# sara-nl/saraGAN

Measured on AMD Instinct MI355X. Metric: 3D volumes/sec/node (G+D step) at 128x128x32, higher is better.
Workload: dtype bf16

## Files before the change

### saragan_amd/csrc/common.h

```cpp
#pragma once
#include <hip/hip_runtime.h>
#include <stdint.h>
#include <mutex>
#include "../../include/saragan_hip.h"

typedef __bf16 bf16_t;
typedef float f32x4 __attribute__((ext_vector_type(4)));
typedef float f32x16 __attribute__((ext_vector_type(16)));
typedef __bf16 bf16x8 __attribute__((ext_vector_type(8)));
typedef __bf16 bf16x4 __attribute__((ext_vector_type(4)));
typedef short s16x4 __attribute__((ext_vector_type(4)));
typedef uint32_t u32x4 __attribute__((ext_vector_type(4)));

#define SG_STORE16_GUARD(v) asm volatile("s_nop 1" ::"v"(v))
typedef uint32_t u32x2 __attribute__((ext_vector_type(2)));

#define SG_LAUNCH_CHECK()                          \
  do {                                             \
    hipError_t e__ = hipGetLastError();            \
    if (e__ != hipSuccess) return (int)e__;        \
  } while (0)

static inline hipStream_t sg_st(sg_stream_t s) { return (hipStream_t)s; }

struct sg_config {
  int fwd_lds, fwd_tg;
  int fwd_v1, fwd_no_pw, fwd_no_dense;
  int fwd_no_v3, fwd_no_v3s, fwd_no_v4, fwd_no_v5, fwd_no_ksplit;
  int fwd3p_16;
  int fwd3s_16;
  int fwd_no_3p;
  int fwd3_gx, fwd3_no_lean;
  int fwd4_gx, fwd4_no_lean, fwd4_no_wres;
  int wgrad_v1, wgrad_no_v3, wgrad_no_lean;
  int wgrad_no_w16;
  int wgrad3l_min_cols;
  int wgrad3l_16;
  int wgrad_v1_blocks;
  int dbg_flags;
  int no_small;
  int deterministic;
  int gemm_ks_model;
  int gemm_k333_maxvox;
  int no_gemm;
};
const sg_config& sg_cfg();

bool sg_gemm_conv_eligible(const sg_conv_shape* s, sg_dtype dt);
size_t sg_gemm_conv_workspace(const sg_conv_shape* s, sg_dtype dt);
int sg_gemm_conv_fwd(const void* x, const void* wp, void* y, const sg_conv_shape* s, const float* bias, int act, float slope,
                     const uint32_t* mask_bits, float mask_slope, uint32_t* sign_out, void* workspace, size_t workspace_bytes,
                     hipStream_t st, bool* used);

bool sg_small_eligible(const sg_conv_shape* s);
bool sg_small_wgrad_eligible(const sg_conv_shape* s);
size_t sg_small_tail_bytes(const sg_conv_shape* s);
size_t sg_small_wgrad_workspace(const sg_conv_shape* s);
int sg_small_pack(const float* w, float coef, int flip, void* tail, const sg_conv_shape* s, sg_dtype dt, hipStream_t st);
int sg_small_fwd(const void* x, const void* tail, void* y, const sg_conv_shape* s, const float* bias, int act, float slope,
                 int pixel_norm, float eps, float* pn_scale, const uint32_t* mask_bits, float mask_slope, uint32_t* sign_out,
                 sg_dtype dt, hipStream_t st);
int sg_small_wgrad(const void* x, const void* dy, float* dw, float* dbias, float coef, void* workspace, size_t workspace_bytes,
                   const sg_conv_shape* s, sg_dtype dt, hipStream_t st);

#define SG_ALLOW_160K_LDS(kern)                                                                                  \
  do {                                                                                                           \
    static std::once_flag once__;                                                                                \
    static hipError_t err__ = hipSuccess;                                                                        \
    std::call_once(once__, [&] {                                                                                 \
      err__ = hipFuncSetAttribute((const void*)(kern), hipFuncAttributeMaxDynamicSharedMemorySize, 160 * 1024);  \
    });                                                                                                          \
    if (err__ != hipSuccess) return (int)err__;                                                                  \
  } while (0)
static inline size_t sg_esize(sg_dtype dt) { return dt == SG_BF16 ? 2 : 4; }
static inline bool sg_aligned16(const void* p) { return (((uintptr_t)p) & 15) == 0; }

__device__ __forceinline__ void philox4x32_10(uint32_t c0, uint32_t c1, uint32_t c2, uint32_t c3, uint32_t k0,
// ... 244 lines not shown
```

### saragan_amd/csrc/conv3d.hip

```cpp
#include "common.h"
#include "prof.h"
#include "conv_args.h"

struct PackArgs {
  const float* w;
  void* wp;
  float coef;
  int taps, kd, kh, kw, cin, cout, nchunk, ntile, flip;
};

template <typename T>
__global__ void pack_weights_kernel(PackArgs a) {
  constexpr int CH = sg_traits<T>::CH;
  constexpr int EPL = CH / 2;
  const int64_t total = (int64_t)a.nchunk * a.taps * a.ntile * 64 * EPL;
  T* out = reinterpret_cast<T*>(a.wp);
  for (int64_t i = (int64_t)blockIdx.x * blockDim.x + threadIdx.x; i < total; i += (int64_t)gridDim.x * blockDim.x) {
    int e = (int)(i % EPL);
    int64_t q = i / EPL;
    int lane = (int)(q % 64); q /= 64;
    int nt = (int)(q % a.ntile); q /= a.ntile;
    int tap = (int)(q % a.taps);
    int chunk = (int)(q / a.taps);
    int ci = chunk * CH + (lane >> 5) * EPL + e;
// ... 11 lines not shown
  }
}

constexpr int SG_PACK_BATCH = 56;
struct PackBatchArgs {
  PackArgs item[SG_PACK_BATCH];
};

template <typename T>
__global__ void pack_weights_batch_kernel(PackBatchArgs b) {
  const PackArgs& a = b.item[blockIdx.y];
  constexpr int CH = sg_traits<T>::CH;
  constexpr int EPL = CH / 2;
  const int64_t total = (int64_t)a.nchunk * a.taps * a.ntile * 64 * EPL;
  T* out = reinterpret_cast<T*>(a.wp);
  for (int64_t i = (int64_t)blockIdx.x * blockDim.x + threadIdx.x; i < total; i += (int64_t)gridDim.x * blockDim.x) {
    int e = (int)(i % EPL);
    int64_t q = i / EPL;
    int lane = (int)(q % 64); q /= 64;
    int nt = (int)(q % a.ntile); q /= a.ntile;
    int tap = (int)(q % a.taps);
    int chunk = (int)(q / a.taps);
    int ci = chunk * CH + (lane >> 5) * EPL + e;
    int co = nt * 32 + (lane & 31);
    float v = 0.f;
    if (ci < a.cin && co < a.cout) {
      v = a.flip ? a.w[((int64_t)(a.taps - 1 - tap) * a.cout + co) * a.cin + ci] : a.w[((int64_t)tap * a.cin + ci) * a.cout + co];
      v *= a.coef;
    }
    out[i] = sg_traits<T>::from_f(v);
  }
}

static inline int conv_nchunk(const sg_conv_shape* s, sg_dtype dt) {
  int ch = dt == SG_BF16 ? 16 : 8;
  return sg_cdiv(s->cin, ch);
}
static inline int conv_ntile(const sg_conv_shape* s) { return sg_cdiv(s->cout, 32); }

static int conv_shape_ok(const sg_conv_shape* s) {
  if (!s) return 0;
  if (s->n < 1 || s->d < 1 || s->h < 1 || s->w < 1 || s->cin < 1 || s->cout < 1) return 0;
  const bool sub = s->kd == 2 && s->kh == 2 && s->kw == 2 && !s->upsample_in;
  if (s->kd < 1 || s->kh < 1 || s->kw < 1 || (!sub && (!(s->kd & 1) || !(s->kh & 1) || !(s->kw & 1)))) return 0;
  if (s->kd > 7 || s->kh > 7 || s->kw > 7) return 0;
  if (s->upsample_in && ((s->d | s->h | s->w) & 1)) return 0;
  return 1;
}

extern "C" size_t sg_conv3d_packed_bytes(const sg_conv_shape* s, sg_dtype dt) {
  if (!conv_shape_ok(s)) return 0;
  return (size_t)conv_nchunk(s, dt) * (s->kd * s->kh * s->kw) * conv_ntile(s) * 1024 + sg_small_tail_bytes(s) + sg_pack16_bytes(s, dt);
}

extern "C" int sg_conv3d_pack_weights(const float* w, float coef, int transpose_flip, void* wp,
                                      const sg_conv_shape* s, sg_dtype dt, sg_stream_t st) {
  if (!conv_shape_ok(s) || !w || !wp) return SG_EINVAL;
  PackArgs a;
  a.w = w; a.wp = wp; a.coef = coef;
  a.kd = s->kd; a.kh = s->kh; a.kw = s->kw; a.taps = s->kd * s->kh * s->kw;
  a.cin = s->cin; a.cout = s->cout; a.nchunk = conv_nchunk(s, dt); a.ntile = conv_ntile(s);
  a.flip = transpose_flip ? 1 : 0;
  int64_t total = (int64_t)a.nchunk * a.taps * a.ntile * 64 * (dt == SG_BF16 ? 8 : 4);
  int blocks = (int)((total + 255) / 256);
  if (blocks > 4096) blocks = 4096;
  if (dt == SG_BF16)
    hipLaunchKernelGGL(pack_weights_kernel<bf16_t>, dim3(blocks), dim3(256), 0, sg_st(st), a);
  else
    hipLaunchKernelGGL(pack_weights_kernel<float>, dim3(blocks), dim3(256), 0, sg_st(st), a);
  SG_LAUNCH_CHECK();
  if (sg_pack16_bytes(s, dt)) {
    void* tail = reinterpret_cast<char*>(wp) + (size_t)a.nchunk * a.taps * a.ntile * 1024;
    return sg_pack16_batch(1, &w, &coef, &a.flip, &tail, s, sg_st(st));
  }
  if (sg_small_tail_bytes(s))
    return sg_small_pack(w, coef, a.flip, reinterpret_cast<char*>(wp) + (size_t)a.nchunk * a.taps * a.ntile * 1024, s, dt, sg_st(st));
  return SG_OK;
}

extern "C" int sg_conv3d_pack_weights_batch(int n, const float* const* w, const float* coef, const int* transpose_flip,
                                            void* const* wp, const sg_conv_shape* shapes, sg_dtype dt, sg_stream_t st) {
  if (n < 0 || (n > 0 && (!w || !coef || !transpose_flip || !wp || !shapes))) return SG_EINVAL;
  if (dt != SG_BF16 && dt != SG_F32) return SG_EINVAL;
  for (int i = 0; i < n; ++i)
    if (!conv_shape_ok(&shapes[i]) || !w[i] || !wp[i]) return SG_EINVAL;
  for (int i0 = 0; i0 < n; i0 += SG_PACK_BATCH) {
    const int m = n - i0 < SG_PACK_BATCH ? n - i0 : SG_PACK_BATCH;
    PackBatchArgs b;
    int64_t most = 0;
    for (int j = 0; j < SG_PACK_BATCH; ++j) {
      const int i = i0 + (j < m ? j : 0);
      const sg_conv_shape* s = &shapes[i];
      PackArgs& a = b.item[j];
      a.w = w[i]; a.wp = wp[i]; a.coef = coef[i];
      a.kd = s->kd; a.kh = s->kh; a.kw = s->kw; a.taps = s->kd * s->kh * s->kw;
      a.cin = s->cin; a.cout = s->cout; a.nchunk = conv_nchunk(s, dt); a.ntile = conv_ntile(s);
      a.flip = transpose_flip[i] ? 1 : 0;
      const int64_t total = (int64_t)a.nchunk * a.taps * a.ntile * 64 * (dt == SG_BF16 ? 8 : 4);
      if (j < m && total > most) most = total;
    }
    int blocks = (int)((most + 255) / 256);
    if (blocks > 256) blocks = 256;
    if (blocks < 1) blocks = 1;
    if (dt == SG_BF16)
      hipLaunchKernelGGL(pack_weights_batch_kernel<bf16_t>, dim3((unsigned)blocks, (unsigned)m), dim3(256), 0, sg_st(st), b);
    else
      hipLaunchKernelGGL(pack_weights_batch_kernel<float>, dim3((unsigned)blocks, (unsigned)m), dim3(256), 0, sg_st(st), b);
    SG_LAUNCH_CHECK();
  }
  constexpr int M16 = 64;
  const float* w16[M16]; float c16[M16]; int f16[M16]; void* d16[M16]; sg_conv_shape s16[M16];
  int n16 = 0;
  for (int i = 0; i < n; ++i) {
    const sg_conv_shape* s = &shapes[i];
    char* tail = reinterpret_cast<char*>(wp[i]) + (size_t)conv_nchunk(s, dt) * (s->kd * s->kh * s->kw) * conv_ntile(s) * 1024;
    int rc = SG_OK;
    if (sg_pack16_bytes(s, dt)) {
      w16[n16] = w[i]; c16[n16] = coef[i]; f16[n16] = transpose_flip[i] ? 1 : 0; d16[n16] = tail; s16[n16] = *s;
      if (++n16 == M16) {
        rc = sg_pack16_batch(n16, w16, c16, f16, d16, s16, sg_st(st));
        n16 = 0;
      }
    } else if (sg_small_tail_bytes(s)) rc = sg_small_pack(w[i], coef[i], transpose_flip[i] ? 1 : 0, tail, s, dt, sg_st(st));
    if (rc != SG_OK) return rc;
  }
  if (n16) return sg_pack16_batch(n16, w16, c16, f16, d16, s16, sg_st(st));
  return SG_OK;
}


template <typename T> struct sg_vec4 { typedef u32x4 type; };
template <> struct sg_vec4<bf16_t> { typedef u32x2 type; };

template <typename T, int MTW, int NTB>
__device__ __forceinline__ void conv_epilogue(f32x16 (&acc)[MTW][NTB], const int64_t (&ooff)[MTW],
                                              const ConvFwdArgs& a, int nt0, int hh) {
  T* y = reinterpret_cast<T*>(a.y);
// ... 2385 lines not shown
    for (int u = 0; u < U; ++u) acc = sg_mfma_chunk<T>(wf[u], xf[u], acc);
  }
#pragma unroll
  for (int i = 0; i < 16; ++i) red[wave][i][lane] = acc[i];
  __syncthreads();
  if (wave == 0) {
#pragma unroll
    for (int i = 0; i < 16; ++i) {
      float t = 0.f;
#pragma unroll
      for (int w = 0; w < 16; ++w) t += red[w][i][lane];
      const int co = nt0 * 32 + (i & 3) + 8 * (i >> 2) + 4 * hh;
      if (a.bias != nullptr && co < a.cout) t += a.bias[co];
      if (a.act) t = fmaxf(t, t * a.slope);
      acc[i] = t;
    }
    if (a.sign_out != nullptr) {
      const uint32_t sw = sg_sign_word(acc, hh);
      if (hh == 0 && vlive) a.sign_out[(int64_t)vrow * a.ntile + nt0] = sw;
    }
    if (a.mask_bits != nullptr && vlive) sg_apply_sign_word(acc, a.mask_bits[(int64_t)vrow * a.ntile + nt0], hh, a.mask_slope);
    if (vlive) {
      T* yrow = reinterpret_cast<T*>(a.y) + (int64_t)vrow * a.cout;
#pragma unroll
      for (int i = 0; i < 16; ++i) {
        const int co = nt0 * 32 + (i & 3) + 8 * (i >> 2) + 4 * hh;
        if (co < a.cout) yrow[co] = sg_traits<T>::from_f(acc[i]);
      }
    }
  }
}

template <typename T>
static int launch_pw_fwd(ConvFwdArgs& a, const sg_conv_shape* s, hipStream_t st, bool* used) {
  *used = false;
  constexpr int E = 16 / (int)sizeof(T);
  if (a.taps != 1 || s->upsample_in || a.pixel_norm) return SG_OK;
  const int64_t nvox = (int64_t)s->n * s->d * s->h * s->w;
  if (nvox <= 128 && s->cin % sg_traits<T>::CH == 0 && a.nchunk >= 64 && !sg_cfg().fwd_no_dense) {
    SG_KNAME("dense_small_m<%s>", sg_tname<T>());
    hipLaunchKernelGGL(dense_small_m_kernel<T>, dim3((unsigned)a.ntile, (unsigned)((nvox + 31) / 32)), dim3(1024), 0, st, a, (int)nvox);
    SG_LAUNCH_CHECK();
    *used = true;
    return SG_OK;
  }
  if (s->cin <= 4 && s->cout % E == 0 && 256 % (s->cout / E) == 0 && s->cout / E <= 256 &&
      ((s->cout / E) & (s->cout / E - 1)) == 0) {
    const int rows = 256 / (s->cout / E);
    const int64_t full = (nvox + rows - 1) / rows;
    int64_t nb = (full + 7) / 8;
    if (nb < 2048) nb = full < 2048 ? full : 2048;
    SG_KNAME("pw_fwd_small_cin<%s>", sg_tname<T>());
    switch (s->cin) {
      case 1: hipLaunchKernelGGL((pw_fwd_small_cin_kernel<T, 1>), dim3((unsigned)nb), dim3(256), 0, st, a, nvox); break;
      case 2: hipLaunchKernelGGL((pw_fwd_small_cin_kernel<T, 2>), dim3((unsigned)nb), dim3(256), 0, st, a, nvox); break;
      case 3: hipLaunchKernelGGL((pw_fwd_small_cin_kernel<T, 3>), dim3((unsigned)nb), dim3(256), 0, st, a, nvox); break;
      default: hipLaunchKernelGGL((pw_fwd_small_cin_kernel<T, 4>), dim3((unsigned)nb), dim3(256), 0, st, a, nvox); break;
    }
    SG_LAUNCH_CHECK();
    *used = true;
  } else if (s->cout <= 4 && s->cin % E == 0 && (s->cin / E) <= 64 && ((s->cin / E) & (s->cin / E - 1)) == 0) {
    const int rows = 256 / (s->cin / E);
    int64_t nb = (nvox + rows - 1) / rows;
    if (nb > 8192) nb = 8192;
    SG_KNAME("pw_fwd_small_cout<%s>", sg_tname<T>());
    hipLaunchKernelGGL(pw_fwd_small_cout_kernel<T>, dim3((unsigned)nb), dim3(256), 0, st, a, nvox);
    SG_LAUNCH_CHECK();
    *used = true;
  }
  return SG_OK;
}

unsigned long long* g_dbg_ts = nullptr;
extern "C" __attribute__((visibility("default"))) void sg_debug_set_ts_buffer(void* p) { g_dbg_ts = (unsigned long long*)p; }

extern "C" size_t sg_conv3d_pw_epilogue_workspace(void) { return (size_t)SG_PW_PART_ROWS * 64 * sizeof(float); }

extern "C" size_t sg_conv3d_fwd_workspace(const sg_conv_shape* s, sg_dtype dt) {
  if (!conv_shape_ok(s) || dt != SG_BF16) return 0;
  if (!sg_cfg().no_gemm && sg_gemm_conv_eligible(s, dt)) return sg_gemm_conv_workspace(s, dt);
  if (s->kd == 3 && s->kh == 3 && s->kw == 3 && s->cin == 64 && s->cout == 32 && s->w % 32 == 0 && s->d >= 4 &&
      (!s->upsample_in || ((s->d | s->h | s->w) & 1) == 0))
    return (size_t)s->n * s->d * s->h * s->w * (size_t)s->cout * 4;
  return 0;
}

extern "C" int sg_conv3d_fwd(const void* x, const void* wp, void* y, const sg_conv_shape* s,
                             const sg_conv_epilogue* ep, sg_dtype dt, sg_stream_t st) {
  if (!conv_shape_ok(s) || !x || !wp || (!y && !(ep && ep->pw_x))) return SG_EINVAL;
  if (ep && ep->struct_size != (uint32_t)sizeof(sg_conv_epilogue)) return SG_EINVAL;
  if (!sg_aligned16(x) || !sg_aligned16(wp) || !sg_aligned16(y)) return SG_EALIGN;
  ConvFwdArgs a;
  a.x = x; a.wp = wp; a.y = y;
  a.bias = ep ? ep->bias : nullptr;
  a.pn_scale = ep ? ep->pn_scale : nullptr;
  a.mask_bits = ep ? reinterpret_cast<const uint32_t*>(ep->mask_bits) : nullptr;
  a.sign_out = ep ? reinterpret_cast<uint32_t*>(ep->sign_out) : nullptr;
  a.mask_slope = ep ? ep->mask_slope : 0.f;
  a.act = ep ? ep->act : 0;
  a.slope = ep ? ep->slope : 0.f;
  a.pixel_norm = ep ? ep->pixel_norm : 0;
  a.eps = ep ? ep->eps : 0.f;
  a.tap_d = ep ? ep->tap_off[0] : 0; a.tap_h = ep ? ep->tap_off[1] : 0; a.tap_w = ep ? ep->tap_off[2] : 0;
  a.pool = ep ? ep->pool : 0;
  if (a.pool < 0 || a.pool > 3) return SG_EINVAL;
  a.pnb_y = ep ? ep->pn_bwd_y : nullptr;
  a.pnb_scale = ep ? ep->pn_bwd_scale : nullptr;
  if ((a.pnb_y != nullptr) != (a.pnb_scale != nullptr) || (a.pnb_y && !sg_aligned16(a.pnb_y))) return SG_EINVAL;
  a.xcs = s->cin; a.xco = 0; a.addend = nullptr;
  a.in_mask = ep ? reinterpret_cast<const uint32_t*>(ep->in_mask_bits) : nullptr;
  a.in_mask_slope = ep ? ep->in_mask_slope : 0.f;
  a.in_gain = ep ? ep->in_gain : 1.f;
// ... 39 lines not shown
    return rc;
  }
  if (a.pool && (subpixel || dt != SG_BF16 || sg_cfg().fwd_v1 || (s->cin * 2) % 16 != 0 || a.pixel_norm ||
                 (a.pool == 1 && (sg_cfg().fwd_no_v3 || sg_cfg().fwd_no_v3s)) || (a.pool == 2 && sg_cfg().fwd_no_v5) ||
                 (a.pool == 3 && (s->cin != 32 || s->kd != 3 || s->kh != 3 || s->kw != 3 || s->upsample_in || !sg_cfg().fwd3s_16 ||
                                  sg_cfg().fwd_no_v3 || sg_cfg().fwd_no_v3s || (ep && ep->x_plane_channels)))))
    return SG_EUNSUPPORTED;
  if (a.pnb_y && (subpixel || dt != SG_BF16 || sg_cfg().fwd_v1 || sg_cfg().fwd_no_v3 || sg_cfg().fwd_no_v3s || a.pool ||
                  a.pixel_norm || (s->cin * 2) % 16 != 0 || s->kd != 3 || s->kh != 3 || s->kw != 3 || s->upsample_in ||
                  (ep && ep->x_plane_channels)))
    return SG_EUNSUPPORTED;
  if (sg_small_eligible(s) && !sg_cfg().no_small && !a.pool && !a.pnb_y && !(ep && ep->x_plane_channels)) {
    rc = sg_small_fwd(x, reinterpret_cast<const char*>(wp) + (size_t)a.nchunk * a.taps * a.ntile * 1024, y, s, a.bias, a.act, a.slope,
                      a.pixel_norm, a.eps, a.pn_scale, a.mask_bits, a.mask_slope, a.sign_out, dt, hs);
    prof.done(rc);
    return rc;
  }
  if (dt == SG_BF16 && !sg_cfg().no_gemm && !a.pool && !a.pnb_y && !a.pixel_norm && !(ep && ep->x_plane_channels) &&
      sg_gemm_conv_eligible(s, dt)) {
    bool used = false;
    rc = sg_gemm_conv_fwd(x, wp, y, s, a.bias, a.act, a.slope, a.mask_bits, a.mask_slope, a.sign_out, ep ? ep->workspace : nullptr,
                          ep ? ep->workspace_bytes : 0, hs, &used);
    if (rc != SG_OK || used) { prof.done(rc); return rc; }
  }
  if (a.pool == 2) {
    bool used = false;
    rc = launch_fwd5(a, s, hs, &used);
    if (rc == SG_OK && !used) rc = SG_EUNSUPPORTED;
    prof.done(rc);
    return rc;
  }
  if (!sg_cfg().fwd_no_pw && !a.pool && !a.pnb_y) {
    bool used = false;
    rc = dt == SG_BF16 ? launch_pw_fwd<bf16_t>(a, s, hs, &used) : launch_pw_fwd<float>(a, s, hs, &used);
    if (rc != SG_OK || used) { prof.done(rc); return rc; }
  }
  const bool v2 = ((s->cin * es) % 16 == 0) && !sg_cfg().fwd_v1;
  const int xpl = ep ? ep->x_plane_channels : 0;
  if (xpl != 0 && (xpl != 32 || s->upsample_in || a.pool || !(v2 && !sg_cfg().fwd_no_v3 && (!a.pixel_norm || a.ntile == 1)))) {
    prof.done(xpl != 32 ? SG_EINVAL : SG_EUNSUPPORTED);
    return xpl != 32 ? SG_EINVAL : SG_EUNSUPPORTED;
  }
  if (v2 && !sg_cfg().fwd_no_v3 && (!a.pixel_norm || a.ntile == 1)) {
    bool used = false;
    rc = SG_OK;
    const bool k333 = s->kd == 3 && s->kh == 3 && s->kw == 3, k133 = s->kd == 1 && s->kh == 3 && s->kw == 3;
    if (dt == SG_BF16 && k333 && !sg_cfg().fwd_no_v3s && !sg_cfg().fwd_no_ksplit && a.nchunk == 4 && a.ntile == 1 && s->cin == 64 &&
        !a.pool && !a.pnb_y && !(a.mask_bits && a.sign_out) && !(a.pixel_norm && a.mask_bits) &&
        !(s->upsample_in && a.mask_bits && !a.in_mask) &&
        !(a.in_mask && (!s->upsample_in || a.sign_out || a.pixel_norm || xpl)) &&
        ep && ep->workspace &&
        ep->workspace_bytes >= (size_t)s->n * s->d * s->h * s->w * (size_t)s->cout * 4 && sg_aligned16(ep->workspace)) {
      if (!sg_cfg().fwd_no_3p && !xpl) {
        bool u3 = false;
        rc = sg_launch_fwd3p(a, s, hs, &u3);
        if (rc != SG_OK || u3) { prof.done(rc); return rc; }
      }
      ConvFwdArgs p1 = a, p2 = a;
      sg_conv_shape sh = *s;
      sh.cin = 32;
      p1.cin = p2.cin = 32; p1.nchunk = p2.nchunk = 2; p1.xcs = p2.xcs = 64;
      p1.xco = 0; p1.y = ep->workspace; p1.bias = nullptr; p1.act = 0; p1.mask_bits = nullptr; p1.sign_out = nullptr;
      p1.pixel_norm = 0; p1.pn_scale = nullptr;
      p2.xco = 32; p2.addend = reinterpret_cast<const float*>(ep->workspace);
      if (xpl) {
        p1.xcs = p2.xcs = 32;
        p2.xco = 0;
// ... 108 lines not shown
```

### saragan_amd/csrc/prof.hip

```cpp
#include "prof.h"
#include <mutex>
#include <vector>
#include <string.h>
#include <stdlib.h>
#include <atomic>

namespace {
struct Rec { int kind; sg_conv_shape shape; int dtype; hipEvent_t e0, e1; bool ok; const char* name; };
std::mutex g_mu;
bool g_on = false;
bool g_filter = false;
int g_fkind = 0;
sg_conv_shape g_fshape;
std::vector<Rec> g_recs;
const char* kVersion = "saragan_hip 0.4 (gfx950)";
}

bool sg_prof_on() { return g_on; }
thread_local const char* sg_tls_kernel = "";

namespace {
std::atomic<const sg_config*> g_cfg{nullptr};
int env_int(const char* name, int dflt) {
  const char* v = getenv(name);
  return v && *v ? atoi(v) : dflt;
}
const sg_config* read_config() {
  sg_config* c = new sg_config;
  c->fwd_lds = env_int("SG_FWD_LDS", 80 * 1024);
  c->fwd_tg = env_int("SG_FWD_TG", 0);
  c->fwd_v1 = env_int("SG_FWD_V1", 0);
  c->fwd_no_pw = env_int("SG_FWD_NO_PW", 0);
  c->fwd_no_dense = env_int("SG_FWD_NO_DENSE", 0);
  c->fwd_no_v3 = env_int("SG_FWD_NO_V3", 0);
  c->fwd_no_v3s = env_int("SG_FWD_NO_V3S", 0);
  c->wgrad_no_lean = env_int("SG_WGRAD_NO_LEAN", 0);
  c->wgrad_no_w16 = env_int("SG_WGRAD_NO_W16", 0);
  c->wgrad3l_16 = env_int("SG_WGRAD3L_16", 0);
  c->wgrad3l_min_cols = env_int("SG_WGRAD3L_MIN_COLS", 0);
  c->wgrad_v1_blocks = env_int("SG_WGRAD_V1_BLOCKS", 0);
  c->fwd_no_v4 = env_int("SG_FWD_NO_V4", 0);
  c->fwd_no_v5 = env_int("SG_FWD_NO_V5", 0);
  c->fwd_no_ksplit = env_int("SG_FWD_NO_KSPLIT", 0);
  c->fwd_no_3p = env_int("SG_FWD_NO_3P", 0);
  c->fwd3p_16 = env_int("SG_FWD3P_16", 1);
  c->fwd3s_16 = env_int("SG_FWD3S_16", 1);
  c->fwd3_gx = env_int("SG_FWD3_GX", 0);
  c->fwd3_no_lean = env_int("SG_FWD3_NO_LEAN", 0);
  c->fwd4_gx = env_int("SG_FWD4_GX", 0);
  c->fwd4_no_lean = env_int("SG_FWD4_NO_LEAN", 0);
  c->fwd4_no_wres = env_int("SG_FWD4_NO_WRES", 0);
  c->wgrad_v1 = env_int("SG_WGRAD_V1", 0);
  c->wgrad_no_v3 = env_int("SG_WGRAD_NO_V3", 0);
  c->dbg_flags = env_int("SG_DBG_FLAGS", 0);
  c->no_small = env_int("SG_NO_SMALL", 0);
  c->deterministic = env_int("SG_DETERMINISTIC", 0);
  c->no_gemm = env_int("SG_NO_GEMM", 0);
  c->gemm_ks_model = env_int("SG_GEMM_KS_MODEL", 0);
  c->gemm_k333_maxvox = env_int("SG_GEMM_K333_MAXVOX", 8192);
  return c;
}
}

const sg_config& sg_cfg() {
  const sg_config* c = g_cfg.load(std::memory_order_acquire);
  if (c == nullptr) {
    std::lock_guard<std::mutex> lk(g_mu);
    c = g_cfg.load(std::memory_order_acquire);
    if (c == nullptr) {
      c = read_config();
      g_cfg.store(c, std::memory_order_release);
    }
  }
  return *c;
}

extern "C" int sg_config_reload(void) {
  std::lock_guard<std::mutex> lk(g_mu);
  g_cfg.store(read_config(), std::memory_order_release);
  return SG_OK;
}

void sg_prof_begin(int kind, const sg_conv_shape* s, sg_dtype dt, hipStream_t st, int* slot) {
  std::lock_guard<std::mutex> lk(g_mu);
  if (g_filter && (kind != g_fkind || memcmp(s, &g_fshape, sizeof(sg_conv_shape)) != 0)) { *slot = -1; return; }
  Rec r; r.kind = kind; r.shape = *s; r.dtype = (int)dt; r.ok = false; r.name = "";
  if (hipEventCreate(&r.e0) != hipSuccess) { *slot = -1; return; }
  if (hipEventCreate(&r.e1) != hipSuccess) { (void)hipEventDestroy(r.e0); *slot = -1; return; }
  (void)hipEventRecord(r.e0, st);
  g_recs.push_back(r);
// ... 84 lines not shown
```

### saragan_amd/csrc/wgrad.hip

```cpp
#include "common.h"
#include "prof.h"
#include <stdlib.h>
#include <type_traits>

struct WgradArgs {
  const void* x;
  const void* dy;
  float* dwt;
  sg_tile_geom g;
  sg_tile_geom gy;
  int cin, cout, taps, kh, kw, tap0, taps_blk;
  int ciT, coT;
  int rs;
  int xbytes, ybytes;
  int ntiles;
  sg_fastdiv fnp;
  int vec_x, vec_y;
  int plane_rows;
  float* dbias;
  int64_t slab, bslab;
  int nslab;
  int dbg_flags;
  unsigned long long* dbg;
  const uint32_t* dy_mask;
// ... 1547 lines not shown
  return vox * (s->cin > s->cout ? s->cin : s->cout) * 2 < (1ll << 31);
}

static int launch_wgrad_planes(WgradArgs& a, const sg_conv_shape* s, hipStream_t st, bool* used) {
  *used = false;
  if (!wgrad_planes_eligible(s)) return SG_OK;
  WgradPlanesArgs p;
  p.x = a.x; p.dy = a.dy; p.dwt = a.dwt; p.dbias = a.dbias; p.cin = s->cin; p.cout = s->cout; p.ciT = a.ciT; p.coT = a.coT;
  p.ntiles = (int)((int64_t)s->n * s->d * s->h * s->w / 128);
  p.slab = a.slab; p.bslab = a.bslab;
  const int pairs = a.ciT * a.coT;
  int gx = sg_cdiv(512, pairs);
  if (gx > 16) gx = 16;
  if (gx > p.ntiles) gx = p.ntiles;
  a.nslab = gx;
  if (s->h == 8) {
    auto kern = conv_wgrad_planes8_kernel;
    SG_ALLOW_160K_LDS(kern);
    SG_KNAME("conv_wgrad_planes<8>");
    constexpr int XB = ((2 * 100 * 4 + 255) / 256) * 4096;
    hipLaunchKernelGGL(kern, dim3((unsigned)gx, (unsigned)pairs), dim3(256), 3 * (size_t)(XB + 8192), st, p);
  } else {
    auto kern = conv_wgrad_planes4_kernel;
    SG_ALLOW_160K_LDS(kern);
    SG_KNAME("conv_wgrad_planes<4>");
    constexpr int XB = ((8 * 36 * 4 + 255) / 256) * 4096;
    hipLaunchKernelGGL(kern, dim3((unsigned)gx, (unsigned)pairs), dim3(256), 3 * (size_t)(XB + 8192), st, p);
  }
  SG_LAUNCH_CHECK();
  *used = true;
  return SG_OK;
}

static size_t wgrad_tile_bytes(const sg_conv_shape* s) {
  const size_t need = (size_t)(s->kd * s->kh * s->kw) * sg_cdiv(s->cin, 32) * sg_cdiv(s->cout, 32) * 4096;
  const bool pointwise = s->kd * s->kh * s->kw == 1 && (s->cin <= 4 || s->cout <= 4);
  const size_t pw = pointwise ? (size_t)PW_WGRAD_MAX_BLOCKS * 5 * (size_t)(s->cin > s->cout ? s->cin : s->cout) * sizeof(float) : 0;
  return ((need > pw ? need : pw) + 255) & ~(size_t)255;
}

extern "C" int sg_conv3d_wgrad(const void* x, const void* dy, float* dw, float coef, void* workspace,
                               size_t workspace_bytes, const sg_conv_shape* s, sg_dtype dt, sg_stream_t st) {
  return sg_conv3d_wgrad_bias(x, dy, dw, nullptr, coef, workspace, workspace_bytes, s, dt, st);
}

static int wgrad_bias_impl(const void* x, const void* dy, float* dw, float* dbias, float coef, void* workspace,
                           size_t workspace_bytes, const sg_conv_shape* s, sg_dtype dt, sg_stream_t st, void* pw_dx,
                           const float* pw_wmat, const void* dy_mask = nullptr, float dy_mask_slope = 0.f, float dy_gain = 1.f,
                           unsigned flags = 0) {
  const int accumulate = (flags & SG_WGRAD_ACCUMULATE) ? 1 : 0;
  const bool clean_ws = (flags & SG_WGRAD_CLEAN_WORKSPACE) != 0;
  if (!conv_shape_ok_w(s) || !x || !dy || !dw || !workspace) return SG_EINVAL;
  if (!sg_aligned16(x) || !sg_aligned16(dy) || !sg_aligned16(workspace)) return SG_EALIGN;
  if (dy_mask && (dt != SG_BF16 || s->kd != 3 || s->kh != 3 || s->kw != 3 || s->upsample_in || (s->cout % 32) ||
                  sg_cfg().wgrad_v1 || sg_cfg().wgrad_no_v3 || !sg_is_pow2f(dy_gain)))
    return SG_EUNSUPPORTED;
  const size_t need = sg_conv3d_wgrad_workspace(s, dt);
  if (workspace_bytes < need) return SG_EWORKSPACE;
  hipStream_t hs = sg_st(st);
  sg_prof_scope prof(1, s, dt, hs);
  {
    const int taps1 = s->kd * s->kh * s->kw;
    const int cs = s->cin < s->cout ? s->cin : s->cout, cb = s->cin < s->cout ? s->cout : s->cin;
    const int E = dt == SG_BF16 ? 8 : 4;
    if (taps1 == 1 && cs <= 4 && !s->upsample_in && cb % E == 0 && cb / E <= 256 && 256 % (cb / E) == 0) {
      if (accumulate || clean_ws) { prof.done(SG_EUNSUPPORTED); return SG_EUNSUPPORTED; }
// ... 4 lines not shown
      const int rows = 256 / (cb / E);
      int64_t nb = (nvox + rows - 1) / rows;
      if (nb > PW_WGRAD_MAX_BLOCKS) nb = PW_WGRAD_MAX_BLOCKS;
      float* part = reinterpret_cast<float*>(workspace);
      const int ones = (dbias != nullptr && small_is_cin) ? 1 : 0;
      SG_KNAME("pw_wgrad_partial");
      if (pw_dx && (!small_is_cin || cb / E > 64)) { prof.done(SG_EUNSUPPORTED); return SG_EUNSUPPORTED; }
      if (dt == SG_BF16 && cs == 1)
        hipLaunchKernelGGL((pw_wgrad_partial_kernel<bf16_t, 1>), dim3((unsigned)nb), dim3(256), 0, hs, (const bf16_t*)sm,
                           (const bf16_t*)bg, part, nvox, cs, cb, ones, (bf16_t*)pw_dx, pw_wmat);
      else if (dt == SG_BF16)
        hipLaunchKernelGGL(pw_wgrad_partial_kernel<bf16_t>, dim3((unsigned)nb), dim3(256), 0, hs, (const bf16_t*)sm,
                           (const bf16_t*)bg, part, nvox, cs, cb, ones, (bf16_t*)pw_dx, pw_wmat);
      else
        hipLaunchKernelGGL(pw_wgrad_partial_kernel<float>, dim3((unsigned)nb), dim3(256), 0, hs, (const float*)sm,
                           (const float*)bg, part, nvox, cs, cb, ones, (float*)pw_dx, pw_wmat);
      hipLaunchKernelGGL(pw_wgrad_final_kernel, dim3((unsigned)(((cs + ones) * cb + 31) / 32)), dim3(256), 0, hs, part,
                         dw, coef, (int)nb, cs, cb, small_is_cin, ones ? dbias : nullptr);
      int e0 = (int)hipGetLastError();
      if (e0 == 0 && dbias && !ones)
        e0 = sg_bias_act_bwd(dy, nullptr, nullptr, dbias, reinterpret_cast<char*>(workspace) + wgrad_tile_bytes(s), nvox,
                             s->cout, 0.f, dt, st);
      prof.done(e0);
      return e0;
    }
  }
  if (pw_dx) { prof.done(SG_EUNSUPPORTED); return SG_EUNSUPPORTED; }
  if (sg_small_wgrad_eligible(s) && !sg_cfg().no_small) {
    if (accumulate || clean_ws) { prof.done(SG_EUNSUPPORTED); return SG_EUNSUPPORTED; }
    const int rc_s = sg_small_wgrad(x, dy, dw, dbias, coef, workspace, workspace_bytes, s, dt, hs);
    prof.done(rc_s);
    return rc_s;
  }
  const size_t tile_bytes = (size_t)(s->kd * s->kh * s->kw) * sg_cdiv(s->cin, 32) * sg_cdiv(s->cout, 32) * 4096;
  const bool det = sg_cfg().deterministic != 0;
  const size_t ns_max = det ? (size_t)wgrad_slab_count(s) : 1;
  hipError_t e = hipSuccess;
  const size_t tile_al = (tile_bytes + 255) & ~(size_t)255;
  float* bias_staged = (!det && dbias) ? reinterpret_cast<float*>(reinterpret_cast<char*>(workspace) + tile_al) : nullptr;
  if (bias_staged && tile_al + (size_t)s->cout * sizeof(float) > ns_max * wgrad_tile_bytes(s) + sg_bias_act_bwd_workspace(s->cout)) {
    prof.done(SG_EWORKSPACE);
    return SG_EWORKSPACE;
  }
  if (!det && !clean_ws)
    e = hipMemsetAsync(workspace, 0, bias_staged ? tile_al + (size_t)s->cout * sizeof(float) : tile_bytes, hs);
  if (e != hipSuccess) { prof.done((int)e); return (int)e; }
  WgradArgs a;
  a.dbias = bias_staged ? bias_staged : dbias;
  a.slab = det ? (int64_t)(wgrad_tile_bytes(s) / 4) : 0;
  a.bslab = det ? (int64_t)(wgrad_bias_slab_bytes(s) / 4) : 0;
  a.nslab = 1;
  float* bias_slabs = reinterpret_cast<float*>(reinterpret_cast<char*>(workspace) + ns_max * wgrad_tile_bytes(s) +
                                               sg_bias_act_bwd_workspace(s->cout));
  if (det && dbias) a.dbias = bias_slabs;
  bool db_done = false;
  a.dbg_flags = sg_cfg().dbg_flags;
  a.dbg = g_dbg_ts;
  a.x = x; a.dy = dy; a.dwt = reinterpret_cast<float*>(workspace);
  a.dy_mask = reinterpret_cast<const uint32_t*>(dy_mask); a.dy_mask_slope = dy_mask_slope; a.dy_gain = dy_gain;
  a.cin = s->cin; a.cout = s->cout;
  a.taps = s->kd * s->kh * s->kw; a.kh = s->kh; a.kw = s->kw;
  a.ciT = sg_cdiv(s->cin, 32); a.coT = sg_cdiv(s->cout, 32);
  int rc = SG_OK;
  bool used = false;
  if (dt == SG_BF16 && !sg_cfg().wgrad_v1 && !sg_cfg().wgrad_no_v3) {
    if (s->kd == 3 && s->kh == 3 && s->kw == 3) rc = launch_wgrad3<3, 3, 3>(a, s, hs, &used);
// ... 75 lines not shown
```

Baseline: 612.7.

## Add vectorized weight packing, split-K dense small-M forward, and dense pointwise wgrad

Adds a new weight-pack kernel in which each thread handles a whole 16-byte fragment, using fast division and vectorized loads on the flipped path. Adds a K-split path for the small-M pointwise forward: partial sums go to workspace slabs and a separate reduce kernel applies the epilogue, which gives more parallelism for wide layers. Adds a direct FP32 dense wgrad kernel for large pointwise layers with few voxels, replacing the tiled wgrad and its workspace memset. These are separate optimizations. The costs are extra kernel launches and workspace traffic, and the bias reduction order changes.

Measured after the change: 616.1, median of 6. No clear change (+0.5%).

```diff
diff --git a/saragan_amd/csrc/common.h b/saragan_amd/csrc/common.h
--- a/saragan_amd/csrc/common.h
+++ b/saragan_amd/csrc/common.h
@@ -43,6 +43,9 @@
   int gemm_ks_model;
   int gemm_k333_maxvox;
   int no_gemm;
+  int fwd_dense_no_ksplit;
+  int pack_v1;
+  int wgrad_no_dense;
 };
 const sg_config& sg_cfg();
 
diff --git a/saragan_amd/csrc/conv3d.hip b/saragan_amd/csrc/conv3d.hip
--- a/saragan_amd/csrc/conv3d.hip
+++ b/saragan_amd/csrc/conv3d.hip
@@ -67,6 +67,80 @@
   }
 }
 
+struct Pack2Args {
+  const float* w;
+  void* wp;
+  float coef;
+  int taps, cin, cout, nchunk, ntile;
+  int flip;
+  uint32_t m1, m2;
+};
+
+template <typename T>
+__device__ __forceinline__ void pack2_item(const Pack2Args& a, int64_t first, int64_t stride) {
+  constexpr int CH = sg_traits<T>::CH;
+  constexpr int EPL = CH / 2;
+  const bool flip = a.flip & 1, vec = a.flip & 2;
+  const sg_fastdiv f1 = {(uint32_t)(flip ? a.nchunk : a.ntile), a.m1}, f2 = {(uint32_t)(flip ? a.ntile : a.taps), a.m2};
+  const int64_t pieces = (int64_t)a.nchunk * a.taps * a.ntile * 64;
+  T* out = reinterpret_cast<T*>(a.wp);
+  for (int64_t i = first; i < pieces; i += stride) {
+    const int lane = (int)(i & 63);
+    const uint32_t f = (uint32_t)(i >> 6);
+    const uint32_t q = sg_div(f, f1), r1 = f - q * f1.d;
+    const uint32_t q2 = sg_div(q, f2), r2 = q - q2 * f2.d;
+    const int chunk = (int)(flip ? r1 : q2), tap = (int)(flip ? q2 : r2), nt = (int)(flip ? r2 : r1);
+    const int ci0 = (int)chunk * CH + (lane >> 5) * EPL;
+    const int co = nt * 32 + (lane & 31);
+    float v[EPL];
+#pragma unroll
+    for (int e = 0; e < EPL; ++e) v[e] = 0.f;
+    if (co < a.cout) {
+      if (!flip) {
+        const float* src = a.w + ((int64_t)tap * a.cin + ci0) * a.cout + co;
+#pragma unroll
+        for (int e = 0; e < EPL; ++e)
+          if (ci0 + e < a.cin) v[e] = src[(int64_t)e * a.cout] * a.coef;
+      } else {
+        const float* src = a.w + ((int64_t)(a.taps - 1 - tap) * a.cout + co) * a.cin + ci0;
+        if (vec && ci0 + EPL <= a.cin) {
+#pragma unroll
+          for (int e4 = 0; e4 < EPL / 4; ++e4) {
+            const f32x4 t = *reinterpret_cast<const f32x4*>(src + 4 * e4);
+#pragma unroll
+            for (int e = 0; e < 4; ++e) v[4 * e4 + e] = t[e] * a.coef;
+          }
+        } else {
+#pragma unroll
+          for (int e = 0; e < EPL; ++e)
+            if (ci0 + e < a.cin) v[e] = src[e] * a.coef;
+        }
+      }
+    }
+    __attribute__((aligned(16))) T tmp[EPL];
+#pragma unroll
+    for (int e = 0; e < EPL; ++e) tmp[e] = sg_traits<T>::from_f(v[e]);
+    const u32x4 t16 = *reinterpret_cast<u32x4*>(tmp);
+    *reinterpret_cast<u32x4*>(out + ((((int64_t)chunk * a.taps + tap) * a.ntile + nt) * 64 + lane) * EPL) = t16;
+    SG_STORE16_GUARD(t16);
+  }
+}
+
+template <typename T>
+__global__ __launch_bounds__(256) void pack_weights2_kernel(Pack2Args b) {
+  pack2_item<T>(b, (int64_t)blockIdx.x * blockDim.x + threadIdx.x, (int64_t)gridDim.x * blockDim.x);
+}
+
+struct Pack2BatchArgs {
+  Pack2Args item[SG_PACK_BATCH];
+};
+static_assert(sizeof(Pack2BatchArgs) <= 4096, "the table travels in the kernel arguments");
+
+template <typename T>
+__global__ __launch_bounds__(256) void pack_weights2_batch_kernel(Pack2BatchArgs b) {
+  pack2_item<T>(b.item[blockIdx.y], (int64_t)blockIdx.x * blockDim.x + threadIdx.x, (int64_t)gridDim.x * blockDim.x);
+}
+
 static inline int conv_nchunk(const sg_conv_shape* s, sg_dtype dt) {
   int ch = dt == SG_BF16 ? 16 : 8;
   return sg_cdiv(s->cin, ch);
@@ -81,6 +155,17 @@
   if (s->kd > 7 || s->kh > 7 || s->kw > 7) return 0;
   if (s->upsample_in && ((s->d | s->h | s->w) & 1)) return 0;
   return 1;
+}
+
+static bool pack2_fill(Pack2Args* a, const float* w, float coef, int flip, void* wp, const sg_conv_shape* s, sg_dtype dt) {
+  a->w = w; a->wp = wp; a->coef = coef;
+  a->taps = s->kd * s->kh * s->kw; a->cin = s->cin; a->cout = s->cout; a->nchunk = conv_nchunk(s, dt); a->ntile = conv_ntile(s);
+  const uint32_t d1 = (uint32_t)(flip ? a->nchunk : a->ntile), d2 = (uint32_t)(flip ? a->ntile : a->taps);
+  const uint64_t nfrag = (uint64_t)a->nchunk * a->taps * a->ntile;
+  if (nfrag * (d1 > d2 ? d1 : d2) >= (1ull << 32)) return false;
+  a->m1 = sg_make_fastdiv(d1).m; a->m2 = sg_make_fastdiv(d2).m;
+  a->flip = flip ? 1 | (s->cin % 4 == 0 && sg_aligned16(w) ? 2 : 0) : 0;
+  return true;
 }
 
 extern "C" size_t sg_conv3d_packed_bytes(const sg_conv_shape* s, sg_dtype dt) {
@@ -97,12 +182,22 @@
   a.cin = s->cin; a.cout = s->cout; a.nchunk = conv_nchunk(s, dt); a.ntile = conv_ntile(s);
   a.flip = transpose_flip ? 1 : 0;
   int64_t total = (int64_t)a.nchunk * a.taps * a.ntile * 64 * (dt == SG_BF16 ? 8 : 4);
-  int blocks = (int)((total + 255) / 256);
-  if (blocks > 4096) blocks = 4096;
-  if (dt == SG_BF16)
-    hipLaunchKernelGGL(pack_weights_kernel<bf16_t>, dim3(blocks), dim3(256), 0, sg_st(st), a);
-  else
-    hipLaunchKernelGGL(pack_weights_kernel<float>, dim3(blocks), dim3(256), 0, sg_st(st), a);
+  Pack2Args a2;
+  if (!sg_cfg().pack_v1 && pack2_fill(&a2, w, coef, a.flip, wp, s, dt)) {
+    int blocks = (int)(((int64_t)a.nchunk * a.taps * a.ntile * 64 + 255) / 256);
+    if (blocks > 4096) blocks = 4096;
+    if (dt == SG_BF16)
+      hipLaunchKernelGGL(pack_weights2_kernel<bf16_t>, dim3(blocks), dim3(256), 0, sg_st(st), a2);
+    else
+      hipLaunchKernelGGL(pack_weights2_kernel<float>, dim3(blocks), dim3(256), 0, sg_st(st), a2);
+  } else {
+    int blocks = (int)((total + 255) / 256);
+    if (blocks > 4096) blocks = 4096;
+    if (dt == SG_BF16)
+      hipLaunchKernelGGL(pack_weights_kernel<bf16_t>, dim3(blocks), dim3(256), 0, sg_st(st), a);
+    else
+      hipLaunchKernelGGL(pack_weights_kernel<float>, dim3(blocks), dim3(256), 0, sg_st(st), a);
+  }
   SG_LAUNCH_CHECK();
   if (sg_pack16_bytes(s, dt)) {
     void* tail = reinterpret_cast<char*>(wp) + (size_t)a.nchunk * a.taps * a.ntile * 1024;
@@ -122,6 +217,8 @@
   for (int i0 = 0; i0 < n; i0 += SG_PACK_BATCH) {
     const int m = n - i0 < SG_PACK_BATCH ? n - i0 : SG_PACK_BATCH;
     PackBatchArgs b;
+    Pack2BatchArgs b2;
+    bool v2 = !sg_cfg().pack_v1;
     int64_t most = 0;
     for (int j = 0; j < SG_PACK_BATCH; ++j) {
       const int i = i0 + (j < m ? j : 0);
@@ -133,11 +230,17 @@
       a.flip = transpose_flip[i] ? 1 : 0;
       const int64_t total = (int64_t)a.nchunk * a.taps * a.ntile * 64 * (dt == SG_BF16 ? 8 : 4);
       if (j < m && total > most) most = total;
-    }
+      v2 = v2 && pack2_fill(&b2.item[j], a.w, a.coef, a.flip, a.wp, s, dt);
+    }
+    if (v2) most /= dt == SG_BF16 ? 8 : 4;
     int blocks = (int)((most + 255) / 256);
     if (blocks > 256) blocks = 256;
     if (blocks < 1) blocks = 1;
-    if (dt == SG_BF16)
+    if (v2 && dt == SG_BF16)
+      hipLaunchKernelGGL(pack_weights2_batch_kernel<bf16_t>, dim3((unsigned)blocks, (unsigned)m), dim3(256), 0, sg_st(st), b2);
+    else if (v2)
+      hipLaunchKernelGGL(pack_weights2_batch_kernel<float>, dim3((unsigned)blocks, (unsigned)m), dim3(256), 0, sg_st(st), b2);
+    else if (dt == SG_BF16)
       hipLaunchKernelGGL(pack_weights_batch_kernel<bf16_t>, dim3((unsigned)blocks, (unsigned)m), dim3(256), 0, sg_st(st), b);
     else
       hipLaunchKernelGGL(pack_weights_batch_kernel<float>, dim3((unsigned)blocks, (unsigned)m), dim3(256), 0, sg_st(st), b);
@@ -2589,14 +2692,144 @@
 }
 
 template <typename T>
-static int launch_pw_fwd(ConvFwdArgs& a, const sg_conv_shape* s, hipStream_t st, bool* used) {
+__device__ __forceinline__ void dense_epilogue(f32x16& acc, const ConvFwdArgs& a, int nt0, int vrow, bool vlive, int hh) {
+#pragma unroll
+  for (int i = 0; i < 16; ++i) {
+    float t = acc[i];
+    const int co = nt0 * 32 + (i & 3) + 8 * (i >> 2) + 4 * hh;
+    if (a.bias != nullptr && co < a.cout) t += a.bias[co];
+    if (a.act) t = fmaxf(t, t * a.slope);
+    acc[i] = t;
+  }
+  if (a.sign_out != nullptr) {
+    const uint32_t sw = sg_sign_word(acc, hh);
+    if (hh == 0 && vlive) a.sign_out[(int64_t)vrow * a.ntile + nt0] = sw;
+  }
+  if (a.mask_bits != nullptr && vlive) sg_apply_sign_word(acc, a.mask_bits[(int64_t)vrow * a.ntile + nt0], hh, a.mask_slope);
+  if (vlive) {
+    T* yrow = reinterpret_cast<T*>(a.y) + (int64_t)vrow * a.cout;
+#pragma unroll
+    for (int i = 0; i < 16; ++i) {
+      const int co = nt0 * 32 + (i & 3) + 8 * (i >> 2) + 4 * hh;
+      if (co < a.cout) yrow[co] = sg_traits<T>::from_f(acc[i]);
+    }
+  }
+}
+
+template <typename T, bool PART>
+__global__ __launch_bounds__(256) void dense_small_m4_kernel(ConvFwdArgs a, int nvox, int cps, float* __restrict__ part) {
+  __shared__ float red[3][16][64];
+  constexpr int CH = sg_traits<T>::CH;
+  const int lane = threadIdx.x & 63, wave = threadIdx.x >> 6;
+  const int r = lane & 31, hh = lane >> 5;
+  const int nt0 = blockIdx.x;
+  const char* wp = reinterpret_cast<const char*>(a.wp) + ((int64_t)nt0 << 10) + lane * 16;
+  const T* x = reinterpret_cast<const T*>(a.x);
+  const int vrow = blockIdx.y * 32 + r;
+  const bool vlive = vrow < nvox;
+  const T* xrow = x + (int64_t)(vlive ? vrow : 0) * a.cin + hh * (CH / 2);
+  const int qb = blockIdx.z * cps, qe = min(a.nchunk, qb + cps);
+  f32x16 acc;
+#pragma unroll
+  for (int i = 0; i < 16; ++i) acc[i] = 0.f;
+  constexpr int U = 8;
+  for (int q0 = qb + wave; q0 < qe; q0 += 4 * U) {
+    u32x4 wf[U], xf[U];
+#pragma unroll
+    for (int u = 0; u < U; ++u) {
+      const int q = q0 + 4 * u;
+      const bool ok = q < qe;
+      wf[u] = ok ? *reinterpret_cast<const u32x4*>(wp + ((int64_t)q * a.ntile << 10)) : u32x4{0u, 0u, 0u, 0u};
+      xf[u] = (ok && vlive) ? *reinterpret_cast<const u32x4*>(xrow + q * CH) : u32x4{0u, 0u, 0u, 0u};
+    }
+#pragma unroll
+    for (int u = 0; u < U; ++u) acc = sg_mfma_chunk<T>(wf[u], xf[u], acc);
+  }
+  if (wave != 0) {
+#pragma unroll
+    for (int i = 0; i < 16; ++i) red[wave - 1][i][lane] = acc[i];
+  }
+  __syncthreads();
+  if (wave != 0) return;
+#pragma unroll
+  for (int i = 0; i < 16; ++i) {
+    float t = acc[i];
+#pragma unroll
+    for (int w = 0; w < 3; ++w) t += red[w][i][lane];
+    acc[i] = t;
+  }
+  if (PART) {
+    float* dst = part + ((((int64_t)blockIdx.z * gridDim.y + blockIdx.y) * a.ntile + nt0) << 10) + lane;
+#pragma unroll
+    for (int i = 0; i < 16; ++i) dst[i * 64] = acc[i];
+  } else {
+    dense_epilogue<T>(acc, a, nt0, vrow, vlive, hh);
+  }
+}
+
+template <typename T>
+__global__ __launch_bounds__(256) void dense_small_m_reduce_kernel(ConvFwdArgs a, int nvox, int nslab, const float* __restrict__ part) {
+  __shared__ float red[16][64];
+  const int lane = threadIdx.x & 63, wave = threadIdx.x >> 6;
+  const int r = lane & 31, hh = lane >> 5;
+  const int nt0 = blockIdx.x;
+  const int64_t slab = ((int64_t)gridDim.y * a.ntile) << 10;
+  const float* src = part + (((int64_t)blockIdx.y * a.ntile + nt0) << 10) + wave * 4 * 64 + lane;
+  float t[4] = {0.f, 0.f, 0.f, 0.f};
+#pragma unroll 4
+  for (int b = 0; b < nslab; ++b) {
+#pragma unroll
+    for (int i = 0; i < 4; ++i) t[i] += src[(int64_t)b * slab + i * 64];
+  }
+#pragma unroll
+  for (int i = 0; i < 4; ++i) red[wave * 4 + i][lane] = t[i];
+  __syncthreads();
+  if (wave != 0) return;
+  f32x16 acc;
+#pragma unroll
+  for (int i = 0; i < 16; ++i) acc[i] = red[i][lane];
+  const int vrow = blockIdx.y * 32 + r;
+  dense_epilogue<T>(acc, a, nt0, vrow, vrow < nvox, hh);
+}
+
+static int dense_ksplit_slabs(int nchunk, int ntile, int rowblocks) {
+  if (nchunk < 256 || sg_cfg().fwd_dense_no_ksplit) return 1;
+  int S = sg_cdiv(256, ntile * rowblocks);
+  if (S > nchunk / 4) S = nchunk / 4;
+  if (S < 2) return 1;
+  return sg_cdiv(nchunk, sg_cdiv(nchunk, S));
+}
+static size_t dense_ksplit_bytes(const sg_conv_shape* s, sg_dtype dt) {
+  const int64_t nvox = (int64_t)s->n * s->d * s->h * s->w;
+  const int ch = dt == SG_BF16 ? 16 : 8;
+  if (s->kd * s->kh * s->kw != 1 || s->upsample_in || nvox > 128 || s->cin % ch != 0 || sg_cfg().fwd_no_dense || sg_cfg().fwd_no_pw) return 0;
+  const int rb = (int)((nvox + 31) / 32), S = dense_ksplit_slabs(conv_nchunk(s, dt), conv_ntile(s), rb);
+  return S > 1 ? (size_t)S * rb * conv_ntile(s) * 4096 : 0;
+}
+
+template <typename T>
+static int launch_pw_fwd(ConvFwdArgs& a, const sg_conv_shape* s, hipStream_t st, bool* used, void* ws = nullptr, size_t ws_bytes = 0) {
   *used = false;
   constexpr int E = 16 / (int)sizeof(T);
   if (a.taps != 1 || s->upsample_in || a.pixel_norm) return SG_OK;
   const int64_t nvox = (int64_t)s->n * s->d * s->h * s->w;
-  if (nvox <= 128 && s->cin % sg_traits<T>::CH == 0 && a.nchunk >= 64 && !sg_cfg().fwd_no_dense) {
+  const bool wide = a.nchunk >= 32 && a.ntile >= 128;
+  if (nvox <= 128 && s->cin % sg_traits<T>::CH == 0 && (a.nchunk >= 64 || wide) && a.ntile <= 65535 && !sg_cfg().fwd_no_dense) {
     SG_KNAME("dense_small_m<%s>", sg_tname<T>());
-    hipLaunchKernelGGL(dense_small_m_kernel<T>, dim3((unsigned)a.ntile, (unsigned)((nvox + 31) / 32)), dim3(1024), 0, st, a, (int)nvox);
+    const int rb = (int)((nvox + 31) / 32);
+    int S = (ws && sg_aligned16(ws)) ? dense_ksplit_slabs(a.nchunk, a.ntile, rb) : 1;
+    if (S > 1 && ws_bytes < (size_t)S * rb * a.ntile * 4096) S = 1;
+    if (S > 1) {
+      hipLaunchKernelGGL((dense_small_m4_kernel<T, true>), dim3((unsigned)a.ntile, (unsigned)rb, (unsigned)S), dim3(256), 0, st, a, (int)nvox,
+                         sg_cdiv(a.nchunk, S), reinterpret_cast<float*>(ws));
+      hipLaunchKernelGGL(dense_small_m_reduce_kernel<T>, dim3((unsigned)a.ntile, (unsigned)rb), dim3(256), 0, st, a, (int)nvox, S,
+                         reinterpret_cast<const float*>(ws));
+    } else if (a.nchunk < 64) {
+      hipLaunchKernelGGL((dense_small_m4_kernel<T, false>), dim3((unsigned)a.ntile, (unsigned)rb, 1u), dim3(256), 0, st, a, (int)nvox,
+                         a.nchunk, (float*)nullptr);
+    } else {
+      hipLaunchKernelGGL(dense_small_m_kernel<T>, dim3((unsigned)a.ntile, (unsigned)rb), dim3(1024), 0, st, a, (int)nvox);
+    }
     SG_LAUNCH_CHECK();
     *used = true;
     return SG_OK;
@@ -2634,7 +2867,9 @@
 extern "C" size_t sg_conv3d_pw_epilogue_workspace(void) { return (size_t)SG_PW_PART_ROWS * 64 * sizeof(float); }
 
 extern "C" size_t sg_conv3d_fwd_workspace(const sg_conv_shape* s, sg_dtype dt) {
-  if (!conv_shape_ok(s) || dt != SG_BF16) return 0;
+  if (!conv_shape_ok(s)) return 0;
+  if (const size_t dense = dense_ksplit_bytes(s, dt)) return dense;
+  if (dt != SG_BF16) return 0;
   if (!sg_cfg().no_gemm && sg_gemm_conv_eligible(s, dt)) return sg_gemm_conv_workspace(s, dt);
   if (s->kd == 3 && s->kh == 3 && s->kw == 3 && s->cin == 64 && s->cout == 32 && s->w % 32 == 0 && s->d >= 4 &&
       (!s->upsample_in || ((s->d | s->h | s->w) & 1) == 0))
@@ -2740,7 +2975,9 @@
   }
   if (!sg_cfg().fwd_no_pw && !a.pool && !a.pnb_y) {
     bool used = false;
-    rc = dt == SG_BF16 ? launch_pw_fwd<bf16_t>(a, s, hs, &used) : launch_pw_fwd<float>(a, s, hs, &used);
+    void* dws = (ep && !ep->pw_x) ? ep->workspace : nullptr;
+    const size_t dwb = dws ? ep->workspace_bytes : 0;
+    rc = dt == SG_BF16 ? launch_pw_fwd<bf16_t>(a, s, hs, &used, dws, dwb) : launch_pw_fwd<float>(a, s, hs, &used, dws, dwb);
     if (rc != SG_OK || used) { prof.done(rc); return rc; }
   }
   const bool v2 = ((s->cin * es) % 16 == 0) && !sg_cfg().fwd_v1;
diff --git a/saragan_amd/csrc/prof.hip b/saragan_amd/csrc/prof.hip
--- a/saragan_amd/csrc/prof.hip
+++ b/saragan_amd/csrc/prof.hip
@@ -56,6 +56,9 @@
   c->no_small = env_int("SG_NO_SMALL", 0);
   c->deterministic = env_int("SG_DETERMINISTIC", 0);
   c->no_gemm = env_int("SG_NO_GEMM", 0);
+  c->fwd_dense_no_ksplit = env_int("SG_DENSE_NO_KSPLIT", 0);
+  c->pack_v1 = env_int("SG_PACK_V1", 0);
+  c->wgrad_no_dense = env_int("SG_WGRAD_NO_DENSE", 0);
   c->gemm_ks_model = env_int("SG_GEMM_KS_MODEL", 0);
   c->gemm_k333_maxvox = env_int("SG_GEMM_K333_MAXVOX", 8192);
   return c;
diff --git a/saragan_amd/csrc/wgrad.hip b/saragan_amd/csrc/wgrad.hip
--- a/saragan_amd/csrc/wgrad.hip
+++ b/saragan_amd/csrc/wgrad.hip
@@ -1603,6 +1603,89 @@
   return SG_OK;
 }
 
+constexpr int WD_CI = 32, WD_CO = 128, WD_V = 32;
+
+template <typename T>
+__global__ __launch_bounds__(256) void conv_wgrad_dense_kernel(const T* __restrict__ x, const T* __restrict__ dy, float* __restrict__ dw,
+                                                               float* __restrict__ dbias, float coef, int rows, int cin, int cout,
+                                                               int accumulate) {
+  constexpr int E = 16 / (int)sizeof(T);
+  constexpr int XP = WD_CI / E, YP = WD_CO / E;
+  __shared__ __attribute__((aligned(16))) float xs[WD_V][WD_CI];
+  __shared__ __attribute__((aligned(16))) float ys[WD_V][WD_CO];
+  const int tid = threadIdx.x;
+  const int ci0 = blockIdx.x * WD_CI, co0 = blockIdx.y * WD_CO;
+  const int tco = (tid & 31) * 4, tci = (tid >> 5) * 4;
+  const bool bias = dbias != nullptr && blockIdx.x == 0 && tid < 32;
+  float acc[4][4];
+#pragma unroll
+  for (int i = 0; i < 4; ++i)
+#pragma unroll
+    for (int j = 0; j < 4; ++j) acc[i][j] = 0.f;
+  float bsum[4] = {0.f, 0.f, 0.f, 0.f};
+  for (int v0 = 0; v0 < rows; v0 += WD_V) {
+    const int vcur = min(WD_V, rows - v0);
+    if (v0) __syncthreads();
+    for (int p = tid; p < vcur * (XP + YP); p += 256) {
+      const int v = p / (XP + YP), q = p - v * (XP + YP);
+      const bool isx = q < XP;
+      const int c = (isx ? q : q - XP) * E;
+      u32x4 raw = {0u, 0u, 0u, 0u};
+      if (isx) raw = *reinterpret_cast<const u32x4*>(x + (int64_t)(v0 + v) * cin + ci0 + c);
+      else if (co0 + c < cout) raw = *reinterpret_cast<const u32x4*>(dy + (int64_t)(v0 + v) * cout + co0 + c);
+      float* dst = isx ? &xs[v][c] : &ys[v][c];
+      const T* el = reinterpret_cast<const T*>(&raw);
+#pragma unroll
+      for (int e = 0; e < E; e += 4) {
+        const f32x4 t = {sg_traits<T>::to_f(el[e]), sg_traits<T>::to_f(el[e + 1]), sg_traits<T>::to_f(el[e + 2]), sg_traits<T>::to_f(el[e + 3])};
+        *reinterpret_cast<f32x4*>(dst + e) = t;
+      }
+    }
+    __syncthreads();
+#pragma unroll 4
+    for (int v = 0; v < vcur; ++v) {
+      const f32x4 xv = *reinterpret_cast<const f32x4*>(&xs[v][tci]);
+      const f32x4 yv = *reinterpret_cast<const f32x4*>(&ys[v][tco]);
+#pragma unroll
+      for (int i = 0; i < 4; ++i)
+#pragma unroll
+        for (int j = 0; j < 4; ++j) acc[i][j] = fmaf(xv[i], yv[j], acc[i][j]);
+      if (bias) {
+#pragma unroll
+        for (int j = 0; j < 4; ++j) bsum[j] += yv[j];
+      }
+    }
+  }
+  const int co = co0 + tco;
+  if (co >= cout) return;
+#pragma unroll
+  for (int i = 0; i < 4; ++i) {
+    float* d = dw + (int64_t)(ci0 + tci + i) * cout + co;
+    f32x4 t;
+#pragma unroll
+    for (int j = 0; j < 4; ++j) t[j] = __fmul_rn(coef, acc[i][j]);
+    if (accumulate) {
+      const f32x4 old = *reinterpret_cast<const f32x4*>(d);
+#pragma unroll
+      for (int j = 0; j < 4; ++j) t[j] = __fadd_rn(old[j], t[j]);
+    }
+    *reinterpret_cast<f32x4*>(d) = t;
+    SG_STORE16_GUARD(t);
+  }
+  if (bias) {
+    const f32x4 t = {bsum[0], bsum[1], bsum[2], bsum[3]};
+    *reinterpret_cast<f32x4*>(dbias + co) = t;
+    SG_STORE16_GUARD(t);
+  }
+}
+
+static bool wgrad_dense_eligible(const sg_conv_shape* s, const float* dw, const float* dbias) {
+  const int64_t rows = (int64_t)s->n * s->d * s->h * s->w;
+  return s->kd * s->kh * s->kw == 1 && !s->upsample_in && rows <= 128 && s->cin % 32 == 0 && s->cout % 32 == 0 &&
+         (int64_t)s->cin * s->cout >= (1 << 20) && s->cout / WD_CO < 65535 && sg_aligned16(dw) && (!dbias || sg_aligned16(dbias)) &&
+         !sg_cfg().wgrad_no_dense;
+}
+
 static size_t wgrad_tile_bytes(const sg_conv_shape* s) {
   const size_t need = (size_t)(s->kd * s->kh * s->kw) * sg_cdiv(s->cin, 32) * sg_cdiv(s->cout, 32) * 4096;
   const bool pointwise = s->kd * s->kh * s->kw == 1 && (s->cin <= 4 || s->cout <= 4);
@@ -1673,6 +1756,22 @@
     prof.done(rc_s);
     return rc_s;
   }
+  if (!dy_mask && !sg_cfg().deterministic && wgrad_dense_eligible(s, dw, dbias)) {
+    const int rows = s->n * s->d * s->h * s->w;
+    const dim3 grid((unsigned)(s->cin / WD_CI), (unsigned)sg_cdiv(s->cout, WD_CO));
+    if (dt == SG_BF16) {
+      SG_KNAME("conv_wgrad_dense<%s>", sg_tname<bf16_t>());
+      hipLaunchKernelGGL(conv_wgrad_dense_kernel<bf16_t>, grid, dim3(256), 0, hs, (const bf16_t*)x, (const bf16_t*)dy, dw, dbias, coef,
+                         rows, s->cin, s->cout, accumulate);
+    } else if (dt == SG_F32) {
+      SG_KNAME("conv_wgrad_dense<%s>", sg_tname<float>());
+      hipLaunchKernelGGL(conv_wgrad_dense_kernel<float>, grid, dim3(256), 0, hs, (const float*)x, (const float*)dy, dw, dbias, coef,
+                         rows, s->cin, s->cout, accumulate);
+    } else { prof.done(SG_EINVAL); return SG_EINVAL; }
+    const int e0 = (int)hipGetLastError();
+    prof.done(e0);
+    return e0;
+  }
   const size_t tile_bytes = (size_t)(s->kd * s->kh * s->kw) * sg_cdiv(s->cin, 32) * sg_cdiv(s->cout, 32) * 4096;
   const bool det = sg_cfg().deterministic != 0;
   const size_t ns_max = det ? (size_t)wgrad_slab_count(s) : 1;
```
